# gargatik/Seamless-Through-Breaking-Rethinking-Image-Stitching-for-Optimal-Alignment

Hardware: AMD Instinct MI355X
Metric: stitched image-pairs/s at 512x512 (higher is better)
Workload: dtype f32 (decoder contractions, PatchEmbed's third conv and the C = 128 block tails: exact 3xbf16 split of both operands, 6 products on the bf16 matrix cores, fp32 accumulate -- error vs fp64 0.83x the fp32 MFMA chain's; everything else fp32); 1 GPU; UDIS-D-shaped 512x512 pairs, batch=1, FlowHomoAdpater.forward(type=test_eval); launch=hipGraph replay, pairs_in_flight=3

## Files before the change

include/stitch_gfx950.h:

```cpp
#ifndef STITCH_GFX950_H
#define STITCH_GFX950_H
#include <stdint.h>
#ifdef __cplusplus
extern "C" {
#endif

typedef struct st_gemm_desc {
    const float* a;
    const float* w;
    float* c;
    const float* bias;
    const float* aux0;
    const float* aux1;
    const float* aux2;
    const float* scale_ptr;
    int32_t M, N, K;
    int32_t H, W, Cin, ldx;
    int32_t kh, kw, sh, sw, ph, pw, Ho, Wo;
    int32_t ldw, ldc, ld_aux0, ld_aux1, ld_aux2;
    int32_t aux0_row_div, aux0_row_mod;
    int32_t act;
    int32_t epi;
    float alpha;
    int32_t batch;
// ... 54 lines not shown
    float* out;
    int32_t lda, ldo, M, nlayers;
    st_chain_layer layer[3];
} st_chain_desc;
int st_linear_chain128(const st_chain_desc* desc, void* stream);
int st_abi_chain_desc_size(void);

typedef struct st_mlp_desc {
    const float* a;
    float* out;
    const float* w1;
    const float* b1;
    const float* w2;
    const float* b2;
    const float* res;
    int32_t lda, ldo, ld_res, M, hidden, ln;
    float ln_eps;
    int32_t reserved;
    const float* wp;
    const float* bp;
    const float* res0;
    int32_t ld_res0, reserved1;
} st_mlp_desc;
int st_mlp128(const st_mlp_desc* desc, void* stream);
int st_abi_mlp_desc_size(void);
int st_mlp128_split3_image_bytes(int32_t hidden, int32_t with_proj, int64_t* bytes);
int st_mlp128_split3_pack(const float* w1, const float* b1, const float* w2, const float* wp, const float* bp, int32_t hidden, void* image,
                          int64_t image_bytes, void* stream);
int st_mlp128_split3(const st_mlp_desc* desc, const void* image, int64_t image_bytes, void* stream);
int st_rowlin128_split3_image_bytes(int32_t N, int64_t* bytes);
int st_rowlin128_split3_pack(const float* w, const float* b, int32_t N, void* image, int64_t image_bytes, void* stream);
int st_rowlin128_split3(const float* a, int32_t lda, float* out, int32_t ldo, int32_t M, int32_t N, int32_t ln, float ln_eps, const void* image,
                        int64_t image_bytes, const float* aux, int32_t ld_aux, int32_t row_div, void* stream);

int st_corr_volume(const float* f1, const float* f2, float* vol, int32_t B, int32_t N1, int32_t N2,
                   int32_t C, void* stream);
int st_corr_volume_both(const float* f1, const float* f2, float* vol12, float* vol21, int32_t B, int32_t N, int32_t C,
                        void* stream);
int st_corr_volume_both_plan(int32_t B, int32_t N, int32_t C, int32_t aligned16);

int st_layernorm(const float* x, int32_t ldx, const float* w, const float* b, float* out, int32_t ldo,
                 int32_t rows, int32_t C, float eps, void* stream);
int st_softmax_rows(float* x, int32_t ld, int32_t rows, int32_t C, void* stream);
int st_l2norm_rows(const float* x, float* out, int32_t rows, int32_t C, void* stream);
int st_maxpool_nhwc(const float* x, float* out, int32_t B, int32_t H, int32_t W, int32_t C, int32_t k,
                    int32_t s, int32_t p, void* stream);
int st_dwconv3x3_residual(const float* x, const float* w, const float* bias, float* out, int32_t B,
                          int32_t H, int32_t W, int32_t C, void* stream);
int st_sine_pe(float* out, int32_t ld, int32_t rows, int32_t dim, const float* coords, int32_t ldc,
               int32_t Wg, int32_t ws, int32_t period, float cscale, float coff, int32_t accumulate,
               void* stream);
int st_attention_small(const float* q, int64_t q_bs, int64_t q_ts, const float* k, int64_t k_bs, int64_t k_ts,
                       const float* v, int64_t v_bs, int64_t v_ts, float* out, int64_t o_bs, int64_t o_ts,
                       int32_t B, int32_t heads, int32_t Nq, int32_t Nk, int32_t D, float scale, void* stream);
int st_attention_kvlds(const float* q, int64_t q_bs, int64_t q_ts, const float* k, int64_t k_bs, int64_t k_ts,
                       const float* v, int64_t v_bs, int64_t v_ts, float* out, int64_t o_bs, int64_t o_ts,
                       int32_t B, int32_t heads, int32_t Nq, int32_t Nk, int32_t D, float scale, void* stream);
int st_window_attention(const float* q, const float* k, const float* v, int64_t bs, int64_t ts,
                        const float* qpad, const float* kpad, const float* vpad, float* out, int64_t o_bs,
                        int64_t o_ts, int32_t B, int32_t H, int32_t W, int32_t heads, int32_t D, int32_t ws,
                        float scale, void* stream);
int st_ccl_softargmax(const float* G, float* out, int32_t ldo, int32_t B, int32_t h, int32_t w, void* stream);
int st_patch_conv1(const float* maps, const float* w36x16, const float* bias, float* out, int32_t M, int32_t H,
                   int32_t W, int32_t Ho, int32_t Wo, void* stream);
int st_patch_conv12(const float* cost_maps, const float* c0_w36x16, const float* c0_b, const float* c2_w32x576,
                    const float* c2_b, float* s2, int32_t M, int32_t H, int32_t W, void* stream);
// ... 178 lines not shown
```

seamless-through-breaking-rethinking-image-stitching-for-optimal-alignment_amd/csrc/common.h:

```cpp
#pragma once
#include <hip/hip_runtime.h>
#include <stdint.h>

#define ST_OK 0
#define ST_EINVAL 1001

#define ST_CHECK_LAUNCH()                         \
    do {                                          \
        hipError_t e__ = hipGetLastError();       \
        if (e__ != hipSuccess) return (int)e__;   \
    } while (0)

__device__ __forceinline__ float st_u8_trunc(float v) { return fminf(fmaxf(truncf(v), 0.f), 255.f); }

enum { ST_ACT_NONE = 0, ST_ACT_RELU = 1, ST_ACT_GELU = 2, ST_ACT_SIGMOID = 3, ST_ACT_TANH = 4, ST_ACT_LRELU = 5 };
enum {
    ST_EPI_STORE = 0,
    ST_EPI_ADD = 1,
    ST_EPI_MUL = 2,
    ST_EPI_GRU = 3,
    ST_EPI_AXPY = 4,
    ST_EPI_ZR = 5
};

// ... 21 lines not shown
    return copysignf((1.0f - e) * __builtin_amdgcn_rcpf(1.0f + e), v);
}
#endif

__device__ __forceinline__ float st_act(float v, int act) {
    switch (act) {
        case ST_ACT_RELU: return v > 0.f ? v : 0.f;
        case ST_ACT_GELU: return st_gelu(v);
        case ST_ACT_SIGMOID: return st_sigmoid(v);
        case ST_ACT_TANH: return st_tanh(v);
        case ST_ACT_LRELU: return v > 0.f ? v : v * 0.01f;
        default: return v;
    }
}

__device__ __forceinline__ float st_logf_cr(float x) { return (float)log((double)x); }

typedef __bf16 bf16x8 __attribute__((ext_vector_type(8)));
__device__ __forceinline__ void st_split3(float x, __bf16& hi, __bf16& mid, __bf16& lo) {
    hi = (__bf16)x;
    float hf = (float)hi;
    if (__builtin_isinf(hf) || hf != hf) {
        if (__builtin_isinf(x) || x != x) { mid = (__bf16)0.f; lo = (__bf16)0.f; return; }
        hf = copysignf(3.3895313892515355e38f, x);
        hi = (__bf16)hf;
    }
    const float r1 = x - hf;
    mid = (__bf16)r1;
    lo = (__bf16)(r1 - (float)mid);
}

__device__ __forceinline__ unsigned short st_bf16_bits(__bf16 v) { return __builtin_bit_cast(unsigned short, v); }

__device__ __forceinline__ float wave_sum(float v) {
#pragma unroll
    for (int o = 32; o > 0; o >>= 1) v += __shfl_xor(v, o, 64);
    return v;
}
__device__ __forceinline__ float wave_max(float v) {
#pragma unroll
    for (int o = 32; o > 0; o >>= 1) v = fmaxf(v, __shfl_xor(v, o, 64));
    return v;
}
```

seamless-through-breaking-rethinking-image-stitching-for-optimal-alignment_amd/csrc/gemm_rows.hip:

```cpp
#include "gemm_common.h"

static bool row_launch_begin(st_gemm_desc& od, int kernel, int tile, void* stream, const float* a, int lda, float* c, int ldc, const void* w, int M, int N,
                             int split3) {
    bool obs = st_observer_installed();
    if (obs) {
        memset(&od, 0, sizeof(od));
        od.a = a; od.c = c; od.w = (const float*)w;
        od.M = M; od.N = N; od.K = 128; od.H = 1; od.W = M; od.Cin = 128; od.ldx = lda; od.ldc = ldc; od.ldw = 128;
        od.kh = od.kw = od.sh = od.sw = 1; od.Ho = 1; od.Wo = M; od.batch = 1; od.alpha = 1.f; od.split3 = split3;
        obs = st_observe(&od, stream, 0);
    }
    st_plan_set(kernel, tile, 1, 1);
    return obs;
}

#define RC_NW 4
__global__ __launch_bounds__(256, 2) void rowchain128_kernel(const st_chain_desc d) {
    constexpr int NJ = 16, NW = RC_NW;
    extern __shared__ __attribute__((aligned(1024))) float smem[];
    float* ring = smem;
    const int tid = threadIdx.x, lane = tid & 63, wave = __builtin_amdgcn_readfirstlane(tid >> 6);
    const int li = lane & 31, lh = lane >> 5;
    const int nblk = (d.M + 31) >> 5;
    const int G = (int)gridDim.x;
// ... 448 lines not shown
extern "C" int st_rowlin128_split3_image_bytes(int32_t N, int64_t* bytes) {
    if (!bytes || N < 32 || N > 4096 || (N & 31)) return ST_EINVAL;
    *bytes = (int64_t)(N / 32) * LS3_STAGE_B;
    return ST_OK;
}
extern "C" int st_rowlin128_split3_pack(const float* w, const float* b, int32_t N, void* image, int64_t image_bytes, void* stream) {
    if (!w || !image || N < 32 || N > 4096 || (N & 31) || ((uintptr_t)image & 15) || image_bytes < (int64_t)(N / 32) * LS3_STAGE_B) return ST_EINVAL;
    hipLaunchKernelGGL(rowlin_split3_pack_kernel, dim3(3, N / 32), dim3(256), 0, (hipStream_t)stream, w, b, (unsigned char*)image);
    ST_CHECK_LAUNCH();
    return ST_OK;
}
extern "C" int st_rowlin128_split3(const float* a, int32_t lda, float* out, int32_t ldo, int32_t M, int32_t N, int32_t ln, float ln_eps, const void* image,
                                   int64_t image_bytes, const float* aux, int32_t ld_aux, int32_t row_div, void* stream) {
    if (aux && (ld_aux < N || (ld_aux & 3) || row_div < 1 || ((uintptr_t)aux & 15) || aux == out)) return ST_EINVAL;
    if (!a || !out || !image || M <= 0 || N < 32 || N > 4096 || (N & 31) || lda < 128 || ldo < N || (lda & 3) || (ldo & 3) || a == out) return ST_EINVAL;
    if ((((uintptr_t)a | (uintptr_t)out | (uintptr_t)image) & 15) || (int64_t)M * (lda > ldo ? lda : ldo) >= ((int64_t)1 << 40)) return ST_EINVAL;
    const int64_t need = (int64_t)(N / 32) * LS3_STAGE_B;
    if (image_bytes < need) return ST_EINVAL;
    const int nblk = (M + 31) / 32;
    int G = (nblk + 3) / 4;
    if (G > 512) G = 512;
    const size_t lds = (size_t)3 * LS3_STAGE_B;
    auto kern = aux ? rowlin128_split3_kernel<true> : rowlin128_split3_kernel<false>;
    (void)hipFuncSetAttribute((const void*)kern, hipFuncAttributeMaxDynamicSharedMemorySize, (int)lds);
    st_gemm_desc od;
    const bool obs = row_launch_begin(od, 10, 40, stream, a, lda, out, ldo, image, M, N, 1);
    hipLaunchKernelGGL(kern, dim3(G), dim3(256), lds, (hipStream_t)stream, a, (int)lda, out, (int)ldo, (int)M, (int)N, (int)ln, ln_eps,
                       (const unsigned char*)image, (unsigned)need, aux, (int)ld_aux, (int)(row_div > 0 ? row_div : 1));
    if (obs) st_observe(&od, stream, 1);
    ST_CHECK_LAUNCH();
    return ST_OK;
}

extern "C" int st_pe_tail_split3_image_bytes(int64_t* bytes) {
    if (!bytes) return ST_EINVAL;
    *bytes = PT3_IMAGE_B;
    return ST_OK;
}
extern "C" int st_pe_tail_split3_pack(const float* w1, int32_t ld1, const float* w2, void* image, int64_t image_bytes, void* stream) {
    if (!w1 || !w2 || !image || ld1 < 64 || ((uintptr_t)image & 15) || image_bytes < PT3_IMAGE_B) return ST_EINVAL;
    hipLaunchKernelGGL(pe_tail_split3_pack_kernel, dim3(3, 4), dim3(256), 0, (hipStream_t)stream, w1, (int)ld1, w2, (unsigned char*)image);
    ST_CHECK_LAUNCH();
    return ST_OK;
}
extern "C" int st_pe_tail_split3(const float* x, const float* tab, int32_t P, const void* image, int64_t image_bytes, const float* b2, const float* gamma,
                                 const float* beta, float eps, float* out, int32_t R, void* stream) {
    if (!x || !tab || !image || !b2 || !gamma || !beta || !out || R <= 0 || P <= 0 || image_bytes < PT3_IMAGE_B || x == out) return ST_EINVAL;
    if ((((uintptr_t)x | (uintptr_t)tab | (uintptr_t)image | (uintptr_t)out) & 15) || (int64_t)R * 128 >= ((int64_t)1 << 40)) return ST_EINVAL;
    const int nblk = (R + 31) / 32;
    int G = (nblk + 3) / 4;
    if (G > 256) G = 256;
    bool tabinv = false;
    for (int g = G; g >= (G > 8 ? G - G / 8 : 1); --g)
        if (((long)g * 128) % P == 0) { G = g; tabinv = true; break; }
    const size_t lds = (size_t)PT3_IMAGE_B + PT3_VEC_B;
    auto kern = tabinv ? pe_tail_split3_kernel<true> : pe_tail_split3_kernel<false>;
    (void)hipFuncSetAttribute((const void*)kern, hipFuncAttributeMaxDynamicSharedMemorySize, (int)lds);
    st_gemm_desc od;
    const bool obs = row_launch_begin(od, 11, 41, stream, x, 64, out, 128, image, R, 192, 1);
    hipLaunchKernelGGL(kern, dim3(G), dim3(256), lds, (hipStream_t)stream, x, tab, (const unsigned char*)image, b2, gamma, beta, eps, out, (int)R, (int)P);
    if (obs) st_observe(&od, stream, 1);
    ST_CHECK_LAUNCH();
    return ST_OK;
}
```

seamless-through-breaking-rethinking-image-stitching-for-optimal-alignment_amd/csrc/mlp_split3.h:

```cpp
#pragma once
#include "gemm_common.h"

#define MS3_W1_B 24576
#define MS3_W2_B 24576
#define MS3_BIAS_B 1024
#define MS3_STAGE_B (MS3_W1_B + MS3_W2_B + MS3_BIAS_B)
#define MS3_PIECES (MS3_STAGE_B / 1024)

typedef __bf16 bf16x2_t __attribute__((ext_vector_type(2)));
typedef float f32x2_t __attribute__((ext_vector_type(2)));

__device__ __forceinline__ unsigned ms3_pk(float a, float b) {
    const f32x2_t v = {a, b};
    return __builtin_bit_cast(unsigned, __builtin_convertvector(v, bf16x2_t));
}
__device__ __forceinline__ void ms3_split_pair(float x0, float x1, unsigned& h, unsigned& m, unsigned& l) {
    h = ms3_pk(x0, x1);
    const float r0 = x0 - __uint_as_float(h << 16), r1 = x1 - __uint_as_float(h & 0xffff0000u);
    m = ms3_pk(r0, r1);
    l = ms3_pk(r0 - __uint_as_float(m << 16), r1 - __uint_as_float(m & 0xffff0000u));
}

__global__ __launch_bounds__(256) void mlp_split3_pack_kernel(const float* __restrict__ w1, const float* __restrict__ b1, const float* __restrict__ w2,
                                                              const float* __restrict__ wp, const float* __restrict__ bp, int hidden,
// ... 435 lines not shown
#pragma unroll
                for (int r = 0; r < 16; ++r) acc[r] = 0.f;
                u32x4 f[3], fn[3];
#pragma unroll
                for (int p = 0; p < 3; ++p) f[p] = *reinterpret_cast<const u32x4*>(ws_ + p * 8192 + fo1[0]);
#pragma unroll
                for (int ks = 0; ks < 8; ++ks) {
                    const int kn = ks + 1 < 8 ? ks + 1 : ks;
#pragma unroll
                    for (int p = 0; p < 3; ++p) fn[p] = *reinterpret_cast<const u32x4*>(ws_ + p * 8192 + fo1[kn]);
                    MS3_SIX(acc, f, xp[0][ks], xp[1][ks], xp[2][ks])
#pragma unroll
                    for (int p = 0; p < 3; ++p) f[p] = fn[p];
                    __builtin_amdgcn_sched_barrier(0);
                }
                const float* bs = reinterpret_cast<const float*>(ws_ + MS3_W1_B);
                float4 v[4];
#pragma unroll
                for (int jj = 0; jj < 4; ++jj) {
                    const float4 bv = *reinterpret_cast<const float4*>(bs + 8 * jj + 4 * lh);
                    v[jj] = make_float4(acc[4 * jj] + bv.x, acc[4 * jj + 1] + bv.y, acc[4 * jj + 2] + bv.z, acc[4 * jj + 3] + bv.w);
                    if (AUX) { v[jj].x += ev[jj].x; v[jj].y += ev[jj].y; v[jj].z += ev[jj].z; v[jj].w += ev[jj].w; }
                }
                if (rok) {
#pragma unroll
                    for (int jj = 0; jj < 4; ++jj) *reinterpret_cast<float4*>(out + rowc * ldo + (c << 5) + 8 * jj + 4 * lh) = v[jj];
                }
            }
            g = g + 1 == 3 ? 0 : g + 1;
        }
    }
}


#define PT3_W1_B 12288
#define PT3_IMAGE_B (4 * PT3_W1_B + 4 * MS3_W2_B)
#define PT3_VEC_B 1536

__global__ __launch_bounds__(256) void pe_tail_split3_pack_kernel(const float* __restrict__ w1, const int ld1, const float* __restrict__ w2, unsigned char* __restrict__ image) {
    const int c = blockIdx.y, t = threadIdx.x;
    bf16x8 h, m, l;
    unsigned char* o;
    if (blockIdx.x == 0) {
        const int r = t >> 3, sl = t & 7, ks = sl >> 1, lh = sl & 1;
#pragma unroll
        for (int e = 0; e < 8; ++e) {
            __bf16 a0, a1, a2;
            st_split3(w1[(size_t)(32 * c + r) * ld1 + 16 * ks + 8 * (e >> 2) + 4 * lh + (e & 3)], a0, a1, a2);
            h[e] = a0; m[e] = a1; l[e] = a2;
        }
        o = image + c * PT3_W1_B + r * 128 + ((sl ^ ((r >> 1) & 7)) << 4);
        *reinterpret_cast<bf16x8*>(o) = h;
        *reinterpret_cast<bf16x8*>(o + 4096) = m;
        *reinterpret_cast<bf16x8*>(o + 8192) = l;
    } else {
        const int idx = (blockIdx.x - 1) * 256 + t, r = idx >> 2, sl = idx & 3, ks = sl >> 1, lh = sl & 1;
#pragma unroll
        for (int e = 0; e < 8; ++e) {
            __bf16 a0, a1, a2;
            st_split3(w2[(size_t)r * 128 + 32 * c + 16 * ks + 8 * (e >> 2) + 4 * lh + (e & 3)], a0, a1, a2);
            h[e] = a0; m[e] = a1; l[e] = a2;
        }
        o = image + 4 * PT3_W1_B + c * MS3_W2_B + r * 64 + ((sl ^ ((r >> 2) & 3)) << 4);
        *reinterpret_cast<bf16x8*>(o) = h;
        *reinterpret_cast<bf16x8*>(o + 8192) = m;
        *reinterpret_cast<bf16x8*>(o + 16384) = l;
// ... 192 lines not shown
```

seamless-through-breaking-rethinking-image-stitching-for-optimal-alignment_amd/csrc/nn.hip:

```cpp
#include "common.h"
#include "../../include/stitch_gfx950.h"

__global__ __launch_bounds__(256) void layernorm_kernel(const float* __restrict__ x, int ldx, const float* __restrict__ w,
                                                        const float* __restrict__ b, float* __restrict__ out, int ldo,
                                                        int rows, int C, float eps) {
    const int row = (blockIdx.x * 256 + threadIdx.x) >> 6, lane = threadIdx.x & 63;
    if (row >= rows) return;
    const float* xr = x + (size_t)row * ldx;
    float v[16];
    float s = 0.f;
#pragma unroll
    for (int i = 0; i < 16; ++i) {
        const int c = lane + 64 * i;
        v[i] = c < C ? xr[c] : 0.f;
        s += v[i];
    }
    const float mean = wave_sum(s) / (float)C;
    float q = 0.f;
#pragma unroll
    for (int i = 0; i < 16; ++i) {
        const int c = lane + 64 * i;
        const float dlt = c < C ? v[i] - mean : 0.f;
        q += dlt * dlt;
    }
// ... 202 lines not shown
    const float v0 = sinf(ax), v1 = cosf(ax), v2 = sinf(ay), v3 = cosf(ay);
    const float val[4] = {v0, v1, v2, v3};
#pragma unroll
    for (int i = 0; i < 4; ++i) {
        const int c = i * q + f;
        if (accumulate == 1 || (accumulate > 1 && c >= accumulate)) o[c] += val[i];
        else o[c] = val[i];
    }
}

extern "C" int st_sine_pe(float* out, int32_t ld, int32_t rows, int32_t dim, const float* coords, int32_t ldc, int32_t Wg,
                          int32_t ws, int32_t period, float cscale, float coff, int32_t accumulate, void* stream) {
    if (!out || rows <= 0 || dim <= 0 || dim % 4 || (!coords && Wg <= 0)) return ST_EINVAL;
    const size_t total = (size_t)rows * (dim / 4);
    hipLaunchKernelGGL(sine_pe_kernel, dim3((total + 255) / 256), dim3(256), 0, (hipStream_t)stream, out, ld, rows, dim,
                       coords, ldc, Wg, ws, period, cscale, coff, accumulate);
    ST_CHECK_LAUNCH();
    return ST_OK;
}

static bool al16(const void* p) { return ((uintptr_t)p & 15) == 0; }

template <int D>
__global__ __launch_bounds__(256) void attention_small_kernel(const float* __restrict__ q, long q_bs, long q_ts,
                                                              const float* __restrict__ k, long k_bs, long k_ts,
                                                              const float* __restrict__ v, long v_bs, long v_ts,
                                                              float* __restrict__ out, long o_bs, long o_ts, int B,
                                                              int heads, int Nq, int Nk, float scale) {
    const long idx = (long)blockIdx.x * 256 + threadIdx.x;
    if (idx >= (long)B * heads * Nq) return;
    const int iq = idx % Nq;
    const int h = (idx / Nq) % heads;
    const int b = idx / ((long)Nq * heads);
    float qr[D], acc[D];
    const float* qp = q + b * q_bs + iq * q_ts + h * D;
#pragma unroll
    for (int e = 0; e < D; e += 4) {
        const float4 t = *reinterpret_cast<const float4*>(qp + e);
        qr[e] = t.x * scale; qr[e + 1] = t.y * scale; qr[e + 2] = t.z * scale; qr[e + 3] = t.w * scale;
    }
    const float* kb = k + b * k_bs + h * D;
    const float* vb = v + b * v_bs + h * D;
    float mx = -INFINITY;
    for (int j = 0; j < Nk; ++j) {
        const float* kp = kb + j * k_ts;
        float s = 0.f;
#pragma unroll
        for (int e = 0; e < D; e += 4) {
            const float4 t = *reinterpret_cast<const float4*>(kp + e);
            s = fmaf(qr[e], t.x, s); s = fmaf(qr[e + 1], t.y, s); s = fmaf(qr[e + 2], t.z, s); s = fmaf(qr[e + 3], t.w, s);
        }
        mx = fmaxf(mx, s);
    }
#pragma unroll
    for (int e = 0; e < D; ++e) acc[e] = 0.f;
    float sum = 0.f;
    for (int j = 0; j < Nk; ++j) {
        const float* kp = kb + j * k_ts;
        float s = 0.f;
#pragma unroll
        for (int e = 0; e < D; e += 4) {
            const float4 t = *reinterpret_cast<const float4*>(kp + e);
            s = fmaf(qr[e], t.x, s); s = fmaf(qr[e + 1], t.y, s); s = fmaf(qr[e + 2], t.z, s); s = fmaf(qr[e + 3], t.w, s);
        }
        const float p = __expf(s - mx);
        sum += p;
        const float* vp = vb + j * v_ts;
#pragma unroll
        for (int e = 0; e < D; e += 4) {
            const float4 t = *reinterpret_cast<const float4*>(vp + e);
            acc[e] = fmaf(p, t.x, acc[e]); acc[e + 1] = fmaf(p, t.y, acc[e + 1]);
            acc[e + 2] = fmaf(p, t.z, acc[e + 2]); acc[e + 3] = fmaf(p, t.w, acc[e + 3]);
        }
    }
    const float inv = 1.0f / sum;
    float* op = out + b * o_bs + iq * o_ts + h * D;
#pragma unroll
    for (int e = 0; e < D; e += 4)
        *reinterpret_cast<float4*>(op + e) = make_float4(acc[e] * inv, acc[e + 1] * inv, acc[e + 2] * inv, acc[e + 3] * inv);
}

extern "C" int st_attention_small(const float* q, int64_t q_bs, int64_t q_ts, const float* k, int64_t k_bs, int64_t k_ts,
                                  const float* v, int64_t v_bs, int64_t v_ts, float* out, int64_t o_bs, int64_t o_ts,
                                  int32_t B, int32_t heads, int32_t Nq, int32_t Nk, int32_t D, float scale, void* stream) {
    if (!q || !k || !v || !out || B <= 0 || heads <= 0 || Nq <= 0 || Nk <= 0) return ST_EINVAL;
    if (!al16(q) || !al16(k) || !al16(v) || !al16(out) || ((q_bs | q_ts | k_bs | k_ts | v_bs | v_ts | o_bs | o_ts) & 3)) return ST_EINVAL;
    const long total = (long)B * heads * Nq;
    dim3 grid((total + 255) / 256), block(256);
    hipStream_t s = (hipStream_t)stream;
#define LAUNCH_AS(DD) hipLaunchKernelGGL(attention_small_kernel<DD>, grid, block, 0, s, q, q_bs, q_ts, k, k_bs, k_ts, v, \
                                         v_bs, v_ts, out, o_bs, o_ts, B, heads, Nq, Nk, scale)
    if (D == 8) LAUNCH_AS(8); else if (D == 16) LAUNCH_AS(16); else if (D == 32) LAUNCH_AS(32); else return ST_EINVAL;
#undef LAUNCH_AS
    ST_CHECK_LAUNCH();
    return ST_OK;
}

typedef float lp_f32x16 __attribute__((ext_vector_type(16)));

__global__ __launch_bounds__(256) void latent_pool_kernel(const float* __restrict__ scores, int ld_s, const float* __restrict__ tokens,
                                                          int ld_t, float* __restrict__ z, int P) {
    const size_t pix = blockIdx.x;
    const int lane = threadIdx.x & 63, wave = threadIdx.x >> 6;
    const int li = lane & 31, lh = lane >> 5;
    const int ib = wave & 1, jb0 = (wave >> 1) * 2;
    const float* Sp = scores + pix * P * ld_s + ib * 32 + li;
    const float* Tp = tokens + pix * P * ld_t + jb0 * 32 + li;
    const int steps = P >> 1;
    float a[32];
    float mx = -INFINITY;
#pragma unroll
    for (int s = 0; s < 32; ++s) {
// ... 633 lines not shown
```

seamless-through-breaking-rethinking-image-stitching-for-optimal-alignment_amd/flowformer.py:

```python
from __future__ import annotations

import os

import torch
import torch.nn as nn

from . import ops
from .checkpoint import HP, ParamTree, flat_params, flow_spec
from .homography import pack_conv


SPLIT3 = os.environ.get("ST_SPLIT3", "1") != "0"


def _new(rows, cols, dev, zero=False):
    return (torch.zeros if zero else torch.empty)((rows, cols), device=dev, dtype=torch.float32)


def _planes_copy(p):
    return ops.Planes(p.rows, p.C, None, t=p.t.clone(), c0=p.c0, ncols=p.ncols)


def _keep(trace, **named):
    if trace is None:
# ... 317 lines not shown

    def _latent_input(self, L, tokens, M, P):
        dev = tokens.device
        lat = self._pk["latents"]
        nl = lat.shape[0]
        att = _new(M * nl, 128, dev)
        if nl == 8 and P % 2 == 0 and P <= 64:
            S = _new(M * P, nl * 8, dev)
            ops.conv_gemm(tokens, L["qfold"], S)
            z = _new(M * nl * 8, 128, dev)
            ops.latent_pool(S, tokens, z, M, P)
            ops.conv_gemm(z.view(M * nl, 8 * 128)[:, :128], L["wv_heads"][:16], att[:, :16], batch=8, bsa=128, bsw=16 * 128, bsc=16)
            proj_b = L["proj_b_fold"]
        else:
            qn = _new(nl, 128, dev)
            ops.layernorm(lat, L["n1"][0], L["n1"][1], qn, 1e-5)
            q = _new(nl, 128, dev)
            ops.conv_gemm(qn, L["q"][0], q, bias=L["q"][1])
            kv = _new(M * P, 256, dev)
            ops.conv_gemm(tokens, L["kv"][0], kv, bias=L["kv"][1])
            ops.attention_small(q, (0, 128), kv[:, :128], (P * 256, 256), kv[:, 128:], (P * 256, 256), att, (nl * 128, 128),
                                M, 8, nl, P, 16, 16 ** -0.5)
            proj_b = L["proj"][1]
        x1 = _new(M * nl, 128, dev)
        ops.conv_gemm(att, L["proj"][0], x1, bias=proj_b, aux0=lat, row_mod=nl)
        o = _new(M * nl, 128, dev)
        if L.get("mlp_s3_plain") is not None:
            return ops.mlp128(x1, o, L["f0_ln"][0], L["f0_ln"][1], L["f3"][0], L["f3"][1], ln_eps=1e-5, image=L["mlp_s3_plain"])
        return ops.linear_chain128(x1, o, [dict(w=L["f0_ln"][0], bias=L["f0_ln"][1], act="gelu", ln_eps=1e-5), dict(w=L["f3"][0], bias=L["f3"][1], res=0)])

    def _latent_self(self, L, x, M):
        dev = x.device
        nl = self._pk["latents"].shape[0]
        qkv = _new(M * nl, 384, dev)
        if L.get("qkv_s3") is not None:
            ops.rowlin128_split3(x, qkv, L["qkv_s3"], ln_eps=1e-5)
        else:
            ops.conv_gemm(x, L["qkv_ln"][0], qkv, bias=L["qkv_ln"][1], ln_eps=1e-5)
        att = _new(M * nl, 128, dev)
        ops.attention_small(qkv[:, :128], (nl * 384, 384), qkv[:, 128:256], (nl * 384, 384), qkv[:, 256:], (nl * 384, 384),
                            att, (nl * 128, 128), M, 8, nl, nl, 16, 16 ** -0.5)
        o = _new(M * nl, 128, dev)
        if L.get("mlp_s3") is not None:
            return ops.mlp128(att, o, L["f0_ln"][0], L["f0_ln"][1], L["f3"][0], L["f3"][1], ln_eps=1e-5, proj=(L["proj"][0], L["proj"][1], x), image=L["mlp_s3"])
        return ops.linear_chain128(att, o, [dict(w=L["proj"][0], bias=L["proj"][1], res=x),
                                            dict(w=L["f0_ln"][0], bias=L["f0_ln"][1], act="gelu", ln_eps=1e-5),
                                            dict(w=L["f3"][0], bias=L["f3"][1], res=1)])

    def _vertical(self, V, x, ctx, B, H1, W1, nl, extra_res=None):
        dev = x.device
        N = H1 * W1
        R = B * N * nl
        C, Cc = 128, 64
        Cq = C + Cc
        y = _new(R, C, dev)
        z = _new(B * N, Cq, dev)
        ops.conv_gemm(ctx, V["lctx"][0], z[:, C:], bias=V["lctx"][1])
        ops.sine_pe(z, Cq, Wg=W1, ws=7, period=N, accumulate=C)
        T = _new(B * N, 3 * C, dev)
        ops.conv_gemm(z, V["ltab"][0], T, bias=V["ltab"][1])
        qkv = _new(R, 3 * C, dev)
        if V.get("lqkv_s3") is not None:
            ops.rowlin128_split3(x, qkv, V["lqkv_s3"], ln_eps=1e-5, aux=T, row_div=nl)
        else:
            ops.conv_gemm(x, V["lqkv_ln"][0], qkv, bias=V["lqkv_ln"][1], aux0=T, row_div=nl, ln_eps=1e-5)
        q, k, v = qkv[:, :C], qkv[:, C:2 * C], qkv[:, 2 * C:]
        key = ("lsa_pad", id(V))
        if key not in self._const:
            zp = _new(49, Cq, dev, zero=True)
            ops.sine_pe(zp, Cq, Wg=7, accumulate=True)
            qp, kp = _new(49, C, dev), _new(49, C, dev)
            ops.conv_gemm(zp, V["lq"][0], qp, bias=V["lq"][1])
            ops.conv_gemm(zp, V["lk"][0], kp, bias=V["lk"][1])
            self._const[key] = (qp, kp, V["lv"][1].expand(49, C).contiguous())
# ... 216 lines not shown
```

seamless-through-breaking-rethinking-image-stitching-for-optimal-alignment_amd/ops.py:

```python
from __future__ import annotations

import ctypes as C

import torch

from ._lib import ChainDesc, GemmDesc, MlpDesc, check, lib
from ._lib import StitchError as StitchErrorBase

ACT = dict(none=0, relu=1, gelu=2, sigmoid=3, tanh=4, lrelu=5)
EPI = dict(store=0, add=1, mul=2, gru=3, axpy=4, zr=5)

assert lib.st_abi_gemm_desc_size() == C.sizeof(GemmDesc), "st_gemm_desc ABI mismatch between header and binding"
assert lib.st_abi_chain_desc_size() == C.sizeof(ChainDesc), "st_chain_desc ABI mismatch between header and binding"
assert lib.st_abi_mlp_desc_size() == C.sizeof(MlpDesc), "st_mlp_desc ABI mismatch between header and binding"


def _stream():
    return C.c_void_p(torch.cuda.current_stream().cuda_stream)


def _p(t):
    if t is None:
        return None
    assert t.is_cuda, "device tensor expected (no CPU fallback)"
# ... 182 lines not shown


def linear_chain128(a, out, layers):
    d = ChainDesc()
    d.a, d.out, d.lda, d.ldo, d.M, d.nlayers = a.data_ptr(), out.data_ptr(), _ld(a), _ld(out), a.shape[0], len(layers)
    for i, y in enumerate(layers):
        ly = d.layer[i]
        w = y["w"]
        assert w.shape == (128, 128) and w.is_contiguous()
        ly.w, ly.bias = w.data_ptr(), (y["bias"].data_ptr() if y.get("bias") is not None else None)
        ly.act = ACT[y.get("act", "none")]
        ly.ln, ly.ln_eps = (1, float(y["ln_eps"])) if y.get("ln_eps") is not None else (0, 0.0)
        r = y.get("res")
        if r is None:
            ly.res = 0
        elif isinstance(r, int):
            ly.res, ly.res_layer = 2, r
        else:
            ly.res, ly.res_ptr, ly.ld_res = 1, r.data_ptr(), _ld(r)
    check(lib.st_linear_chain128(C.byref(d), _stream()), "st_linear_chain128")
    return out


def rowlin128_split3_pack(w, b):
    N = w.shape[0]
    assert w.shape == (N, 128) and w.is_contiguous() and (b is None or b.shape == (N,))
    nb = C.c_int64(0)
    check(lib.st_rowlin128_split3_image_bytes(N, C.byref(nb)), "st_rowlin128_split3_image_bytes")
    img = torch.empty(nb.value, dtype=torch.uint8, device=w.device)
    check(lib.st_rowlin128_split3_pack(_p(w), _p(b), N, C.c_void_p(img.data_ptr()), nb.value, _stream()), "st_rowlin128_split3_pack")
    return img


def rowlin128_split3(a, out, image, ln_eps=None, aux=None, row_div=1):
    assert a.shape[1] == 128 and out.shape[0] == a.shape[0] and out.shape[1] % 32 == 0
    if aux is not None:
        assert aux.shape[1] == out.shape[1] and aux.shape[0] * row_div >= a.shape[0]
    check(lib.st_rowlin128_split3(_p(a), _ld(a), _p(out), _ld(out), a.shape[0], out.shape[1], 1 if ln_eps is not None else 0,
                                  float(ln_eps or 0.0), C.c_void_p(image.data_ptr()), image.numel(), _p(aux), _ld(aux) if aux is not None else 0, row_div,
                                  _stream()), "st_rowlin128_split3")
    return out


def mlp128_split3_pack(w1, b1, w2, proj=None):
    hidden = w1.shape[0]
    assert w1.shape == (hidden, 128) and w2.shape == (128, hidden) and w1.is_contiguous() and w2.is_contiguous() and b1.shape == (hidden,)
    nb = C.c_int64(0)
    check(lib.st_mlp128_split3_image_bytes(hidden, 1 if proj is not None else 0, C.byref(nb)), "st_mlp128_split3_image_bytes")
    img = torch.empty(nb.value, dtype=torch.uint8, device=w1.device)
    wp, bp = proj if proj is not None else (None, None)
    if wp is not None:
        assert wp.shape == (128, 128) and wp.is_contiguous()
    check(lib.st_mlp128_split3_pack(_p(w1), _p(b1), _p(w2), _p(wp) if wp is not None else None, _p(bp) if bp is not None else None, hidden,
                                    C.c_void_p(img.data_ptr()), nb.value, _stream()), "st_mlp128_split3_pack")
    return img


def mlp128(a, out, w1, b1, w2, b2, ln_eps=None, res=None, proj=None, image=None):
    hidden = w1.shape[0]
    assert w1.shape == (hidden, 128) and w2.shape == (128, hidden) and w1.is_contiguous() and w2.is_contiguous()
    assert b1.shape == (hidden,) and b2.shape == (128,) and a.shape[1] == 128 and out.shape == a.shape
    d = MlpDesc()
    d.a, d.out, d.lda, d.ldo, d.M, d.hidden = a.data_ptr(), out.data_ptr(), _ld(a), _ld(out), a.shape[0], hidden
    d.w1, d.b1, d.w2, d.b2 = w1.data_ptr(), b1.data_ptr(), w2.data_ptr(), b2.data_ptr()
    d.ln, d.ln_eps = (1, float(ln_eps)) if ln_eps is not None else (0, 0.0)
    if res is not None:
# ... 840 lines not shown
```

Measured before the change: 97.63 pairs/s.

## Fuse latent self-attention QKV projection with per-row 8-latent attention in one kernel

Adds a kernel that computes the LayerNorm + split3 bf16 QKV projection for latent rows and immediately runs the 8-latent, 8-head attention in registers. K and V are exchanged between lanes with ds_bpermute, so the 384-wide qkv intermediate never goes to global memory and one launch is saved. Weights are streamed through LDS with a triple-buffered buffer_load-to-LDS pipeline. The existing attention_small kernel is refactored onto a shared row-head helper. The cost is a more complex, register-heavy kernel that only applies when there are 8 latents.

```diff
diff --git a/include/stitch_gfx950.h b/include/stitch_gfx950.h
--- a/include/stitch_gfx950.h
+++ b/include/stitch_gfx950.h
@@ -110,6 +110,8 @@
 int st_rowlin128_split3_pack(const float* w, const float* b, int32_t N, void* image, int64_t image_bytes, void* stream);
 int st_rowlin128_split3(const float* a, int32_t lda, float* out, int32_t ldo, int32_t M, int32_t N, int32_t ln, float ln_eps, const void* image,
                         int64_t image_bytes, const float* aux, int32_t ld_aux, int32_t row_div, void* stream);
+int st_latent_qkv_attn_split3(const float* a, int32_t lda, float* out, int32_t ldo, int32_t M, int32_t ln, float ln_eps, const void* image,
+                              int64_t image_bytes, float scale, void* stream);
 
 int st_corr_volume(const float* f1, const float* f2, float* vol, int32_t B, int32_t N1, int32_t N2,
                    int32_t C, void* stream);
diff --git a/seamless-through-breaking-rethinking-image-stitching-for-optimal-alignment_amd/csrc/common.h b/seamless-through-breaking-rethinking-image-stitching-for-optimal-alignment_amd/csrc/common.h
--- a/seamless-through-breaking-rethinking-image-stitching-for-optimal-alignment_amd/csrc/common.h
+++ b/seamless-through-breaking-rethinking-image-stitching-for-optimal-alignment_amd/csrc/common.h
@@ -77,6 +77,57 @@
 
 __device__ __forceinline__ unsigned short st_bf16_bits(__bf16 v) { return __builtin_bit_cast(unsigned short, v); }
 
+template <int D, int NK, class KLoad, class VLoad>
+__device__ __forceinline__ void st_attn_row_head(const float (&q)[D], const float scale, const int nk, KLoad kload, VLoad vload, float (&out)[D]) {
+    float qr[D], acc[D];
+#pragma unroll
+    for (int e = 0; e < D; ++e) qr[e] = q[e] * scale;
+    auto score = [&](int j) {
+        float t[D];
+        kload(j, t);
+        float s = 0.f;
+#pragma unroll
+        for (int e = 0; e < D; ++e) s = fmaf(qr[e], t[e], s);
+        return s;
+    };
+    auto accumulate = [&](int j, float s, float mx, float& sum) {
+        const float p = __expf(s - mx);
+        sum += p;
+        float t[D];
+        vload(j, t);
+#pragma unroll
+        for (int e = 0; e < D; ++e) acc[e] = fmaf(p, t[e], acc[e]);
+    };
+#pragma unroll
+    for (int e = 0; e < D; ++e) acc[e] = 0.f;
+    float mx = -INFINITY, sum = 0.f;
+    if constexpr (NK > 0) {
+        float sk[NK];
+#pragma unroll
+        for (int i = 0; i < NK; ++i) sk[i] = 0.f;
+#pragma unroll 1
+        for (int j = 0; j < NK; ++j) {
+            const float s = score(j);
+            mx = fmaxf(mx, s);
+#pragma unroll
+            for (int i = 0; i + 1 < NK; ++i) sk[i] = sk[i + 1];
+            sk[NK - 1] = s;
+        }
+#pragma unroll 1
+        for (int j = 0; j < NK; ++j) {
+            accumulate(j, sk[0], mx, sum);
+#pragma unroll
+            for (int i = 0; i + 1 < NK; ++i) sk[i] = sk[i + 1];
+        }
+    } else {
+        for (int j = 0; j < nk; ++j) mx = fmaxf(mx, score(j));
+        for (int j = 0; j < nk; ++j) accumulate(j, score(j), mx, sum);
+    }
+    const float inv = 1.0f / sum;
+#pragma unroll
+    for (int e = 0; e < D; ++e) out[e] = acc[e] * inv;
+}
+
 __device__ __forceinline__ float wave_sum(float v) {
 #pragma unroll
     for (int o = 32; o > 0; o >>= 1) v += __shfl_xor(v, o, 64);
diff --git a/seamless-through-breaking-rethinking-image-stitching-for-optimal-alignment_amd/csrc/gemm_rows.hip b/seamless-through-breaking-rethinking-image-stitching-for-optimal-alignment_amd/csrc/gemm_rows.hip
--- a/seamless-through-breaking-rethinking-image-stitching-for-optimal-alignment_amd/csrc/gemm_rows.hip
+++ b/seamless-through-breaking-rethinking-image-stitching-for-optimal-alignment_amd/csrc/gemm_rows.hip
@@ -504,6 +504,26 @@
     return ST_OK;
 }
 
+extern "C" int st_latent_qkv_attn_split3(const float* a, int32_t lda, float* out, int32_t ldo, int32_t M, int32_t ln, float ln_eps, const void* image,
+                                         int64_t image_bytes, float scale, void* stream) {
+    if (!a || !out || !image || M <= 0 || (M & 7) || lda < 128 || ldo < 128 || (lda & 3) || (ldo & 3) || a == out) return ST_EINVAL;
+    if ((((uintptr_t)a | (uintptr_t)out | (uintptr_t)image) & 15) || (int64_t)M * (lda > ldo ? lda : ldo) >= ((int64_t)1 << 40)) return ST_EINVAL;
+    const int64_t need = (int64_t)LQA_STEPS * LS3_STAGE_B;
+    if (image_bytes < need) return ST_EINVAL;
+    const int nblk = (M + 31) / 32;
+    int G = (nblk + 3) / 4;
+    if (G > 512) G = 512;
+    const size_t lds = (size_t)3 * LS3_STAGE_B;
+    (void)hipFuncSetAttribute((const void*)latent_qkv_attn_split3_kernel, hipFuncAttributeMaxDynamicSharedMemorySize, (int)lds);
+    st_gemm_desc od;
+    const bool obs = row_launch_begin(od, 12, 42, stream, a, lda, out, ldo, image, M, 384, 1);
+    hipLaunchKernelGGL(latent_qkv_attn_split3_kernel, dim3(G), dim3(256), lds, (hipStream_t)stream, a, (int)lda, out, (int)ldo, (int)M, (int)ln, ln_eps,
+                       (const unsigned char*)image, (unsigned)need, scale);
+    if (obs) st_observe(&od, stream, 1);
+    ST_CHECK_LAUNCH();
+    return ST_OK;
+}
+
 extern "C" int st_pe_tail_split3_image_bytes(int64_t* bytes) {
     if (!bytes) return ST_EINVAL;
     *bytes = PT3_IMAGE_B;
diff --git a/seamless-through-breaking-rethinking-image-stitching-for-optimal-alignment_amd/csrc/mlp_split3.h b/seamless-through-breaking-rethinking-image-stitching-for-optimal-alignment_amd/csrc/mlp_split3.h
--- a/seamless-through-breaking-rethinking-image-stitching-for-optimal-alignment_amd/csrc/mlp_split3.h
+++ b/seamless-through-breaking-rethinking-image-stitching-for-optimal-alignment_amd/csrc/mlp_split3.h
@@ -491,6 +491,171 @@
     }
 }
 
+#define LQA_STEPS 12
+#pragma clang diagnostic push
+#pragma clang diagnostic ignored "-Winline-asm"
+
+__device__ __forceinline__ void lqa_head_of_lane(const float4 (&v)[4], float (&h)[16]) {
+#pragma unroll
+    for (int u = 0; u < 2; ++u) {
+        const float a[4] = {v[u].x, v[u].y, v[u].z, v[u].w}, b[4] = {v[u + 2].x, v[u + 2].y, v[u + 2].z, v[u + 2].w};
+#pragma unroll
+        for (int t = 0; t < 4; ++t) {
+            const auto r = __builtin_amdgcn_permlane32_swap(__float_as_uint(a[t]), __float_as_uint(b[t]), false, false);
+            h[8 * u + t] = __uint_as_float(r[0]);
+            h[8 * u + 4 + t] = __uint_as_float(r[1]);
+        }
+    }
+}
+
+__global__ __launch_bounds__(256, 2) void latent_qkv_attn_split3_kernel(const float* __restrict__ a, const int lda, float* __restrict__ out, const int ldo,
+                                                                        const int M, const int ln, const float ln_eps, const unsigned char* __restrict__ image,
+                                                                        const unsigned image_bytes, const float scale) {
+    extern __shared__ __attribute__((aligned(1024))) unsigned char sm3[];
+    const int tid = threadIdx.x, lane = tid & 63, wave = __builtin_amdgcn_readfirstlane(tid >> 6);
+    const int li = lane & 31, lh = lane >> 5;
+    const int nblk = (M + 31) >> 5;
+    const int G = (int)gridDim.x;
+    const int blk0 = (int)blockIdx.x * 4;
+    const int rounds = blk0 < nblk ? (nblk - blk0 + G * 4 - 1) / (G * 4) : 0;
+    const int total = rounds * LQA_STEPS;
+    if (total == 0) return;
+    const unsigned lds0 = (unsigned)(size_t)(__attribute__((address_space(3))) unsigned char*)sm3;
+    const i32x4 rsd = make_rsrc(image, image_bytes);
+    const unsigned vlin = (unsigned)lane << 4;
+    int c_dma = 0, w_dma = 0, g_dma = 0, q_dma = 0;
+    auto dma_step = [&]() {
+        const unsigned dst = lds0 + (unsigned)(g_dma * LS3_STAGE_B), src = (unsigned)((w_dma * 4 + c_dma) * LS3_STAGE_B), o = (unsigned)wave * 6144u;
+        asm volatile("s_mov_b32 m0, %0\n\ts_nop 0\n\t"
+                     "buffer_load_dwordx4 %1, %2, %3 offen lds\n\t"
+                     "buffer_load_dwordx4 %1, %2, %3 offen offset:1024 lds\n\t"
+                     "buffer_load_dwordx4 %1, %2, %3 offen offset:2048 lds\n\t"
+                     "buffer_load_dwordx4 %1, %2, %3 offen offset:3072 lds"
+                     : : "s"(dst + o), "v"(vlin), "s"(rsd), "s"(src + o) : "memory", "m0");
+        asm volatile("s_mov_b32 m0, %0\n\ts_nop 0\n\t"
+                     "buffer_load_dwordx4 %1, %2, %3 offen lds\n\t"
+                     "buffer_load_dwordx4 %1, %2, %3 offen offset:1024 lds"
+                     : : "s"(dst + o + 4096u), "v"(vlin), "s"(rsd), "s"(src + o + 4096u) : "memory", "m0");
+        if (wave == 0)
+            asm volatile("s_mov_b32 m0, %0\n\ts_nop 0\n\t"
+                         "buffer_load_dwordx4 %1, %2, %3 offen lds"
+                         : : "s"(dst + (unsigned)MS3_W1_B), "v"(vlin), "s"(rsd), "s"(src + (unsigned)MS3_W1_B) : "memory", "m0");
+        ++q_dma;
+        if (++w_dma == 3) { w_dma = 0; c_dma = c_dma + 1 == 4 ? 0 : c_dma + 1; }
+        g_dma = g_dma + 1 == 3 ? 0 : g_dma + 1;
+    };
+    dma_step();
+    dma_step();
+    int fo1[8];
+#pragma unroll
+    for (int ks = 0; ks < 8; ++ks) fo1[ks] = li * 256 + (((2 * ks + lh) ^ (li & 15)) << 4);
+    int g = 0;
+    for (int rd = 0; rd < rounds; ++rd) {
+        const int blk = blk0 + wave + rd * G * 4;
+        const bool active = blk < nblk;
+        const int row = blk * 32 + li;
+        const bool rok = active && row < M;
+        const size_t rowc = (size_t)(active && row < M ? row : M - 1);
+        u32x4 xp[3][8];
+        if (active) {
+            float4 x[16];
+#pragma unroll
+            for (int j = 0; j < 16; ++j) x[j] = *reinterpret_cast<const float4*>(a + rowc * lda + 8 * j + 4 * lh);
+            if (ln) {
+                float s = 0.f;
+#pragma unroll
+                for (int j = 0; j < 16; ++j) s += (x[j].x + x[j].y) + (x[j].z + x[j].w);
+                s += __shfl_xor(s, 32, 64);
+                const float mean = s * (1.0f / 128.0f);
+                float v = 0.f;
+#pragma unroll
+                for (int j = 0; j < 16; ++j) {
+                    x[j].x -= mean; x[j].y -= mean; x[j].z -= mean; x[j].w -= mean;
+                    v += (x[j].x * x[j].x + x[j].y * x[j].y) + (x[j].z * x[j].z + x[j].w * x[j].w);
+                }
+                v += __shfl_xor(v, 32, 64);
+                const float rstd = 1.0f / sqrtf(v * (1.0f / 128.0f) + ln_eps);
+#pragma unroll
+                for (int j = 0; j < 16; ++j) { x[j].x *= rstd; x[j].y *= rstd; x[j].z *= rstd; x[j].w *= rstd; }
+            }
+#pragma unroll
+            for (int j = 0; j < 16; ++j) {
+                unsigned h0, m0, l0, h1, m1, l1;
+                ms3_split_pair(x[j].x, x[j].y, h0, m0, l0);
+                ms3_split_pair(x[j].z, x[j].w, h1, m1, l1);
+                xp[0][j >> 1][2 * (j & 1)] = h0; xp[0][j >> 1][2 * (j & 1) + 1] = h1;
+                xp[1][j >> 1][2 * (j & 1)] = m0; xp[1][j >> 1][2 * (j & 1) + 1] = m1;
+                xp[2][j >> 1][2 * (j & 1)] = l0; xp[2][j >> 1][2 * (j & 1) + 1] = l1;
+            }
+        }
+        __builtin_amdgcn_sched_barrier(0);
+        auto step = [&](float4 (&v)[4], const bool stored) {
+            if (stored && active) asm volatile("s_waitcnt vmcnt(4)" ::: "memory");
+            else asm volatile("s_waitcnt vmcnt(0)" ::: "memory");
+            __syncthreads();
+            if (q_dma < total) dma_step();
+            if (active) {
+                const unsigned char* ws_ = sm3 + g * LS3_STAGE_B;
+                f32x16 acc;
+#pragma unroll
+                for (int r = 0; r < 16; ++r) acc[r] = 0.f;
+                u32x4 f[3], fn[3];
+#pragma unroll
+                for (int p = 0; p < 3; ++p) f[p] = *reinterpret_cast<const u32x4*>(ws_ + p * 8192 + fo1[0]);
+#pragma unroll
+                for (int ks = 0; ks < 8; ++ks) {
+                    const int kn = ks + 1 < 8 ? ks + 1 : ks;
+#pragma unroll
+                    for (int p = 0; p < 3; ++p) fn[p] = *reinterpret_cast<const u32x4*>(ws_ + p * 8192 + fo1[kn]);
+                    MS3_SIX(acc, f, xp[0][ks], xp[1][ks], xp[2][ks])
+#pragma unroll
+                    for (int p = 0; p < 3; ++p) f[p] = fn[p];
+                    __builtin_amdgcn_sched_barrier(0);
+                }
+                const float* bs = reinterpret_cast<const float*>(ws_ + MS3_W1_B);
+#pragma unroll
+                for (int jj = 0; jj < 4; ++jj) {
+                    const float4 bv = *reinterpret_cast<const float4*>(bs + 8 * jj + 4 * lh);
+                    v[jj] = make_float4(acc[4 * jj] + bv.x, acc[4 * jj + 1] + bv.y, acc[4 * jj + 2] + bv.z, acc[4 * jj + 3] + bv.w);
+                }
+            }
+            g = g + 1 == 3 ? 0 : g + 1;
+        };
+#pragma unroll 1
+        for (int c = 0; c < 4; ++c) {
+            float4 vq[4], vk[4], vv[4];
+            step(vq, c > 0);
+            step(vk, false);
+            step(vv, false);
+            if (active) {
+                float qh[16], kh[16], vh[16], oh[16];
+                lqa_head_of_lane(vq, qh);
+                lqa_head_of_lane(vk, kh);
+                lqa_head_of_lane(vv, vh);
+                st_attn_row_head<16, 8>(
+                    qh, scale, 8,
+                    [&](int j, float (&t)[16]) {
+                        const int src = ((lane & 56) + j) << 2;
+#pragma unroll
+                        for (int e = 0; e < 16; ++e) t[e] = __int_as_float(__builtin_amdgcn_ds_bpermute(src, __float_as_int(kh[e])));
+                    },
+                    [&](int j, float (&t)[16]) {
+                        const int src = ((lane & 56) + j) << 2;
+#pragma unroll
+                        for (int e = 0; e < 16; ++e) t[e] = __int_as_float(__builtin_amdgcn_ds_bpermute(src, __float_as_int(vh[e])));
+                    },
+                    oh);
+                if (rok) {
+                    float* op = out + rowc * ldo + (c << 5) + 16 * lh;
+#pragma unroll
+                    for (int e = 0; e < 16; e += 4) *reinterpret_cast<float4*>(op + e) = make_float4(oh[e], oh[e + 1], oh[e + 2], oh[e + 3]);
+                }
+            }
+        }
+    }
+}
+#pragma clang diagnostic pop
+
 
 #define PT3_W1_B 12288
 #define PT3_IMAGE_B (4 * PT3_W1_B + 4 * MS3_W2_B)
diff --git a/seamless-through-breaking-rethinking-image-stitching-for-optimal-alignment_amd/csrc/nn.hip b/seamless-through-breaking-rethinking-image-stitching-for-optimal-alignment_amd/csrc/nn.hip
--- a/seamless-through-breaking-rethinking-image-stitching-for-optimal-alignment_amd/csrc/nn.hip
+++ b/seamless-through-breaking-rethinking-image-stitching-for-optimal-alignment_amd/csrc/nn.hip
@@ -258,52 +258,26 @@
     const int iq = idx % Nq;
     const int h = (idx / Nq) % heads;
     const int b = idx / ((long)Nq * heads);
-    float qr[D], acc[D];
+    float qv[D], o[D];
     const float* qp = q + b * q_bs + iq * q_ts + h * D;
 #pragma unroll
     for (int e = 0; e < D; e += 4) {
         const float4 t = *reinterpret_cast<const float4*>(qp + e);
-        qr[e] = t.x * scale; qr[e + 1] = t.y * scale; qr[e + 2] = t.z * scale; qr[e + 3] = t.w * scale;
+        qv[e] = t.x; qv[e + 1] = t.y; qv[e + 2] = t.z; qv[e + 3] = t.w;
     }
     const float* kb = k + b * k_bs + h * D;
     const float* vb = v + b * v_bs + h * D;
-    float mx = -INFINITY;
-    for (int j = 0; j < Nk; ++j) {
-        const float* kp = kb + j * k_ts;
-        float s = 0.f;
+    auto row = [](const float* p, float (&t)[D]) {
 #pragma unroll
         for (int e = 0; e < D; e += 4) {
-            const float4 t = *reinterpret_cast<const float4*>(kp + e);
-            s = fmaf(qr[e], t.x, s); s = fmaf(qr[e + 1], t.y, s); s = fmaf(qr[e + 2], t.z, s); s = fmaf(qr[e + 3], t.w, s);
-        }
-        mx = fmaxf(mx, s);
-    }
-#pragma unroll
-    for (int e = 0; e < D; ++e) acc[e] = 0.f;
-    float sum = 0.f;
-    for (int j = 0; j < Nk; ++j) {
-        const float* kp = kb + j * k_ts;
-        float s = 0.f;
-#pragma unroll
-        for (int e = 0; e < D; e += 4) {
-            const float4 t = *reinterpret_cast<const float4*>(kp + e);
-            s = fmaf(qr[e], t.x, s); s = fmaf(qr[e + 1], t.y, s); s = fmaf(qr[e + 2], t.z, s); s = fmaf(qr[e + 3], t.w, s);
-        }
-        const float p = __expf(s - mx);
-        sum += p;
-        const float* vp = vb + j * v_ts;
-#pragma unroll
-        for (int e = 0; e < D; e += 4) {
-            const float4 t = *reinterpret_cast<const float4*>(vp + e);
-            acc[e] = fmaf(p, t.x, acc[e]); acc[e + 1] = fmaf(p, t.y, acc[e + 1]);
-            acc[e + 2] = fmaf(p, t.z, acc[e + 2]); acc[e + 3] = fmaf(p, t.w, acc[e + 3]);
-        }
-    }
-    const float inv = 1.0f / sum;
+            const float4 f = *reinterpret_cast<const float4*>(p + e);
+            t[e] = f.x; t[e + 1] = f.y; t[e + 2] = f.z; t[e + 3] = f.w;
+        }
+    };
+    st_attn_row_head<D, 0>(qv, scale, Nk, [&](int j, float (&t)[D]) { row(kb + j * k_ts, t); }, [&](int j, float (&t)[D]) { row(vb + j * v_ts, t); }, o);
     float* op = out + b * o_bs + iq * o_ts + h * D;
 #pragma unroll
-    for (int e = 0; e < D; e += 4)
-        *reinterpret_cast<float4*>(op + e) = make_float4(acc[e] * inv, acc[e + 1] * inv, acc[e + 2] * inv, acc[e + 3] * inv);
+    for (int e = 0; e < D; e += 4) *reinterpret_cast<float4*>(op + e) = make_float4(o[e], o[e + 1], o[e + 2], o[e + 3]);
 }
 
 extern "C" int st_attention_small(const float* q, int64_t q_bs, int64_t q_ts, const float* k, int64_t k_bs, int64_t k_ts,
diff --git a/seamless-through-breaking-rethinking-image-stitching-for-optimal-alignment_amd/flowformer.py b/seamless-through-breaking-rethinking-image-stitching-for-optimal-alignment_amd/flowformer.py
--- a/seamless-through-breaking-rethinking-image-stitching-for-optimal-alignment_amd/flowformer.py
+++ b/seamless-through-breaking-rethinking-image-stitching-for-optimal-alignment_amd/flowformer.py
@@ -373,14 +373,17 @@
     def _latent_self(self, L, x, M):
         dev = x.device
         nl = self._pk["latents"].shape[0]
-        qkv = _new(M * nl, 384, dev)
-        if L.get("qkv_s3") is not None:
-            ops.rowlin128_split3(x, qkv, L["qkv_s3"], ln_eps=1e-5)
-        else:
-            ops.conv_gemm(x, L["qkv_ln"][0], qkv, bias=L["qkv_ln"][1], ln_eps=1e-5)
         att = _new(M * nl, 128, dev)
-        ops.attention_small(qkv[:, :128], (nl * 384, 384), qkv[:, 128:256], (nl * 384, 384), qkv[:, 256:], (nl * 384, 384),
-                            att, (nl * 128, 128), M, 8, nl, nl, 16, 16 ** -0.5)
+        if L.get("qkv_s3") is not None and nl == 8:
+            ops.latent_qkv_attn_split3(x, att, L["qkv_s3"], 16 ** -0.5, ln_eps=1e-5)
+        else:
+            qkv = _new(M * nl, 384, dev)
+            if L.get("qkv_s3") is not None:
+                ops.rowlin128_split3(x, qkv, L["qkv_s3"], ln_eps=1e-5)
+            else:
+                ops.conv_gemm(x, L["qkv_ln"][0], qkv, bias=L["qkv_ln"][1], ln_eps=1e-5)
+            ops.attention_small(qkv[:, :128], (nl * 384, 384), qkv[:, 128:256], (nl * 384, 384), qkv[:, 256:], (nl * 384, 384),
+                                att, (nl * 128, 128), M, 8, nl, nl, 16, 16 ** -0.5)
         o = _new(M * nl, 128, dev)
         if L.get("mlp_s3") is not None:
             return ops.mlp128(att, o, L["f0_ln"][0], L["f0_ln"][1], L["f3"][0], L["f3"][1], ln_eps=1e-5, proj=(L["proj"][0], L["proj"][1], x), image=L["mlp_s3"])
diff --git a/seamless-through-breaking-rethinking-image-stitching-for-optimal-alignment_amd/ops.py b/seamless-through-breaking-rethinking-image-stitching-for-optimal-alignment_amd/ops.py
--- a/seamless-through-breaking-rethinking-image-stitching-for-optimal-alignment_amd/ops.py
+++ b/seamless-through-breaking-rethinking-image-stitching-for-optimal-alignment_amd/ops.py
@@ -238,6 +238,14 @@
     return img
 
 
+def latent_qkv_attn_split3(a, out, image, scale, ln_eps=None):
+    assert a.shape[1] == 128 and out.shape == (a.shape[0], 128), (a.shape, out.shape)
+    check(lib.st_latent_qkv_attn_split3(_p(a), _ld(a), _p(out), _ld(out), a.shape[0], 1 if ln_eps is not None else 0,
+                                        float(ln_eps or 0.0), C.c_void_p(image.data_ptr()), image.numel(), float(scale), _stream()),
+          "st_latent_qkv_attn_split3")
+    return out
+
+
 def rowlin128_split3(a, out, image, ln_eps=None, aux=None, row_div=1):
     assert a.shape[1] == 128 and out.shape[0] == a.shape[0] and out.shape[1] % 32 == 0
     if aux is not None:
```

New measurement: 98.45 pairs/s (median of 6 runs). Within noise of the previous version (+0.8%).
